# moribots/plen_ml_walk

Hardware: NVIDIA B200
Metric: PLEN env-steps/sec (higher is better)
Workload: dtype f32

## Files before the change

### plen_ml_walk_b200/csrc/plen_device.cuh

```cuda
#pragma once

#include <math.h>
#include <stdint.h>

#include "../../include/plen_b200.h"

#ifndef PLEN_HOST_EMU
#define PLEN_DEV __device__ __forceinline__
#define PLEN_DEV_NOINLINE __device__ __noinline__
namespace plen {
PLEN_DEV int lane_id() { return threadIdx.x & 31; }
PLEN_DEV float shfl(float v, int src) { return __shfl_sync(0xffffffffu, v, src); }
PLEN_DEV float shfl4(float v, int src) { return __shfl_sync(0xffffffffu, v, src, 4); }
PLEN_DEV float shfl_up(float v, int d) { return __shfl_up_sync(0xffffffffu, v, d); }
PLEN_DEV float shfl_down(float v, int d) { return __shfl_down_sync(0xffffffffu, v, d); }
PLEN_DEV float shfl_xor(float v, int m) { return __shfl_xor_sync(0xffffffffu, v, m); }
PLEN_DEV unsigned ballot(bool p) { return __ballot_sync(0xffffffffu, p); }
PLEN_DEV unsigned redux_max(unsigned v) { return __reduce_max_sync(0xffffffffu, v); }
PLEN_DEV unsigned redux_or(unsigned v) { return __reduce_or_sync(0xffffffffu, v); }
PLEN_DEV void warp_sync() { __syncwarp(); }
PLEN_DEV float f_as_u_max(float v) { return __uint_as_float(redux_max(__float_as_uint(v))); }
PLEN_DEV void sincos_(float x, float *s, float *c) { sincosf(x, s, c); }
#ifndef PLEN_FAST_RCP
#define PLEN_FAST_RCP 1
#endif
PLEN_DEV float rcp_(float x) {
#if PLEN_FAST_RCP
    float r;
    asm("rcp.approx.ftz.f32 %0, %1;" : "=f"(r) : "f"(x));
    return r;
#else
    return 1.0f / x;
#endif
}
PLEN_DEV unsigned f_bits(float v) { return __float_as_uint(v); }
PLEN_DEV int lowest_bit(unsigned m) { return __ffs((int)m) - 1; }
PLEN_DEV int highest_bit(unsigned m) { return 31 - __clz((int)m); }
PLEN_DEV int popc_(unsigned m) { return __popc(m); }
}
#endif

namespace plen {

enum {
    T_RPJ = 0, T_PPJ = 9, T_AXIS = 12, T_COM = 15, T_MASS = 18, T_INERTIA = 19, T_LOWER = 25, T_UPPER = 26,
    T_CS = 27, T_CE = 28, T_ENVLO = 29, T_ENVHI = 30,
    T_BOX_LANE = 31, T_BOX_C = 32, T_BOX_R = 35, T_BOX_H = 44, T_BOX_REST = 47, T_ROWS = 48
};

enum {
    W_U = 0,
    W_Q = 32,
    W_POS = 32,
    W_MAN = 35,
    W_EPRET = 36,
    W_QUAT = 56,
    W_CNT = 60, W_DS = 61, W_HIST = 62, W_EPT = 63,
    W_LAST = 64,
    W_SUMS = 70,
    W_ITERS = 79,
    W_SPARE = 80
};

struct DevConfig {
    float dt, inv_dt, gravity_z, motor_imp, kp_over_dt, one_minus_kd, linear_damping;
    float mu_lateral, mu_spinning, mu_rolling, restitution, rest_thresh, erp_contact_over_dt, erp_joint_over_dt;
    float linear_slop, warm, hull_margin, vmax, residual_threshold, mu_link;
    float foot_break[2];
    float foot_pts[2][4][3];
    float start_pos[3];
    int foot_lane[2];
    int substeps, reset_ticks, iterations, joint_act, max_episode_steps, auto_reset, link_contacts, n_boxes;
    int sole_manifold, n_hull[2];
    const float *hull;
    float support_tie;
};

enum {
    SR_G = 0,
    SR_B = 960,
    SR_MRHS = 1152, SR_MD = 1184, SR_LDIR = 1216, SR_LRHS = 1248, SR_VSTAR = 1280, SR_Q = 1312,
    SR_CRHS = 1344, SR_CDINV = 1408, SR_CD = 1472,
    SR_PT = 1536,
    SR_LAMC = 1568,
    SR_BASE = 1576,
    SR_WORDS = 1600
};

enum {
    XR_NX = 0,
    XR_ROWS = 16,
    XR_J = 0, XR_B = 32, XR_BB = 64, XR_RHS = 70, XR_DINV = 71, XR_D = 72, XR_ROW_WORDS = 80,
    XR_WORDS = XR_ROWS + 3 * PLEN_MAX_BOX_POINTS * XR_ROW_WORDS
};
#define PLEN_KEY_EXT 125

PLEN_DEV int nth_bit4(unsigned m, int k) {
    int r = -1, c = 0;
#pragma unroll
    for (int b = 0; b < 4; b++) {
        const bool on = (m >> b) & 1u;
        r = (on && c == k) ? b : r;
        c += on ? 1 : 0;
    }
    return r;
}

#ifndef PLEN_HOST_EMU
struct __align__(16) vec4 { float x, y, z, w; };
struct __align__(8) vec2 { float x, y; };
#define PLEN_ALIGN16 __align__(16)
#else
struct vec4 { float x, y, z, w; };
struct vec2 { float x, y; };
#define PLEN_ALIGN16
#endif

#ifndef PLEN_HOST_EMU
PLEN_DEV float gld(const float *p) {
    float v;
    asm("ld.global.f32 %0, [%1];" : "=f"(v) : "l"(p));
    return v;
}
PLEN_DEV vec4 gld4(const float *p) {
    vec4 r;
    asm("ld.global.v4.f32 {%0, %1, %2, %3}, [%4];" : "=f"(r.x), "=f"(r.y), "=f"(r.z), "=f"(r.w) : "l"(p));
    return r;
}
PLEN_DEV int gld_i(const int *p) {
    int v;
    asm("ld.global.s32 %0, [%1];" : "=r"(v) : "l"(p));
    return v;
}
PLEN_DEV int gld_u8(const uint8_t *p) {
    unsigned v;
    asm("ld.global.u8 %0, [%1];" : "=r"(v) : "l"(p));
    return (int)v;
}
#else
PLEN_DEV float gld(const float *p) { return *p; }
PLEN_DEV vec4 gld4(const float *p) { return *reinterpret_cast<const vec4 *>(p); }
PLEN_DEV int gld_i(const int *p) { return *p; }
PLEN_DEV int gld_u8(const uint8_t *p) { return *p; }
#endif

PLEN_DEV void load6(const float *row, float (&o)[6]) {
    const vec4 a = *reinterpret_cast<const vec4 *>(row);
    const vec2 b = *reinterpret_cast<const vec2 *>(row + 4);
    o[0] = a.x; o[1] = a.y; o[2] = a.z; o[3] = a.w; o[4] = b.x; o[5] = b.y;
}

struct PLEN_ALIGN16 WarpScratch {
    float st[96];
    float tw[24][8];
    float kk[24][8];
    float gg[24][8];
    float cb[32];
    float minv[24][32];
    float cp[8][4];
    union {
        float lin[12][12];
        float red[32 * 21];
    };
    float obs[32];
    float xp[PLEN_MAX_BOX_POINTS][8];
    float mn[2][28];
    float mlam[8];
};

struct LaneState {
    float u;
    float q;
    float tgt;
    float lam;
    float pos[3];
    float quat[4];
    unsigned man;
    int iters;
    float fric_s, motor_s, kp_s;
};

PLEN_DEV void mat3_mul(const float *A, const float *B, float *C) {
#pragma unroll
    for (int i = 0; i < 3; i++)
#pragma unroll
        for (int j = 0; j < 3; j++) C[3 * i + j] = A[3 * i] * B[j] + A[3 * i + 1] * B[3 + j] + A[3 * i + 2] * B[6 + j];
}
PLEN_DEV void mat3_vec(const float *A, const float *v, float *o) {
    o[0] = A[0] * v[0] + A[1] * v[1] + A[2] * v[2];
    o[1] = A[3] * v[0] + A[4] * v[1] + A[5] * v[2];
    o[2] = A[6] * v[0] + A[7] * v[1] + A[8] * v[2];
}
PLEN_DEV void cross(const float *a, const float *b, float *o) {
    o[0] = a[1] * b[2] - a[2] * b[1];
    o[1] = a[2] * b[0] - a[0] * b[2];
    o[2] = a[0] * b[1] - a[1] * b[0];
}
PLEN_DEV void quat_to_mat(const float *q, float *R) {
    const float x = q[0], y = q[1], z = q[2], w = q[3];
    R[0] = 1 - 2 * (y * y + z * z); R[1] = 2 * (x * y - w * z); R[2] = 2 * (x * z + w * y);
    R[3] = 2 * (x * y + w * z); R[4] = 1 - 2 * (x * x + z * z); R[5] = 2 * (y * z - w * x);
    R[6] = 2 * (x * z - w * y); R[7] = 2 * (y * z + w * x); R[8] = 1 - 2 * (x * x + y * y);
}
PLEN_DEV float warp_sum(float v) {
#pragma unroll
    for (int m = 16; m > 0; m >>= 1) v += shfl_xor(v, m);
    return v;
}
PLEN_DEV void warp_sum2(float &a, float &b) {
#pragma unroll
    for (int m = 16; m > 0; m >>= 1) { a += shfl_xor(a, m); b += shfl_xor(b, m); }
}

PLEN_DEV void forward_kinematics(const float *tab, int lane, float q, const float *quat, float *Rw, float *pw) {
    float R[9], p[3];
    {
        float s, c;
        sincos_(q, &s, &c);
        const float ax = tab[(T_AXIS + 0) * 32 + lane], ay = tab[(T_AXIS + 1) * 32 + lane], az = tab[(T_AXIS + 2) * 32 + lane];
        const float t = 1.0f - c;
        float Rq[9] = {t * ax * ax + c, t * ax * ay - s * az, t * ax * az + s * ay,
                       t * ax * ay + s * az, t * ay * ay + c, t * ay * az - s * ax,
                       t * ax * az - s * ay, t * ay * az + s * ax, t * az * az + c};
        float Rpj[9];
#pragma unroll
        for (int k = 0; k < 9; k++) Rpj[k] = tab[(T_RPJ + k) * 32 + lane];
        mat3_mul(Rpj, Rq, R);
#pragma unroll
        for (int k = 0; k < 3; k++) p[k] = tab[(T_PPJ + k) * 32 + lane];
    }
    const int cs = (int)tab[T_CS * 32 + lane];
#pragma unroll
    for (int d = 1; d < 8; d <<= 1) {
        float Rp[9], pp[3];
#pragma unroll
        for (int k = 0; k < 9; k++) Rp[k] = shfl_up(R[k], d);
#pragma unroll
        for (int k = 0; k < 3; k++) pp[k] = shfl_up(p[k], d);
        if (lane - d >= cs) {
            float t[3], Rn[9];
            mat3_vec(Rp, p, t);
            p[0] = pp[0] + t[0]; p[1] = pp[1] + t[1]; p[2] = pp[2] + t[2];
            mat3_mul(Rp, R, Rn);
#pragma unroll
            for (int k = 0; k < 9; k++) R[k] = Rn[k];
        }
    }
    float R0[9];
    quat_to_mat(quat, R0);
    mat3_mul(R0, R, Rw);
    mat3_vec(R0, p, pw);
}

PLEN_DEV float clampf(float x, float lo, float hi) { return fminf(fmaxf(x, lo), hi); }

PLEN_DEV void row_entries(int type, const float *a, const float *m, const float *Y, float px, float py, float pz,
                          float &J, float &B) {
    switch (type) {
        case 0: J = a[0] * py - a[1] * px + m[2]; B = Y[0] * py - Y[1] * px + Y[5]; break;
        case 1: J = a[2]; B = Y[2]; break;
        case 2: J = -a[1]; B = -Y[1]; break;
        case 3: J = a[0]; B = Y[0]; break;
        case 4: J = a[0] * pz - a[2] * px - m[1]; B = Y[0] * pz - Y[2] * px - Y[4]; break;
        default: J = a[1] * pz - a[2] * py + m[0]; B = Y[1] * pz - Y[2] * py + Y[3]; break;
    }
}

struct DebugOut { float *minv, *pos, *rot; };

PLEN_DEV_NOINLINE void box_rows(const DevConfig &cfg, const float *tab, WarpScratch &ws, int lane, float vstar, int nx, float *srx);
PLEN_DEV_NOINLINE int box_points(const DevConfig &cfg, const float *tab, WarpScratch &ws, int lane, bool touch, float cz, float rz0,
                                 float rz1, float rz2, int bl, float R0, float R1, float R2, float R3, float R4, float R5, float R6,
                                 float R7, float R8, float p0, float p1, float p2);

PLEN_DEV_NOINLINE void manifold_merge(const DevConfig &cfg, float *mn, float *lam, const float *Rf, const float *pf, const float *pos,
                                      int f, int idx);

PLEN_DEV_NOINLINE unsigned sole_manifold_contacts(const DevConfig &cfg, WarpScratch &ws, int lane, float *man, float pos0, float pos1,
                                                  float pos2, float lam_in, float R0, float R1, float R2, float R3, float R4, float R5,
                                                  float R6, float R7, float R8, float p0, float p1, float p2);

PLEN_DEV void tick_dynamics(const DevConfig &cfg, const float *tab, WarpScratch &ws, LaneState &L, int lane,
                            float *srec, uint8_t *sort_key, const DebugOut *dbg = nullptr, float *srx = nullptr,
                            float *man = nullptr) {
    const bool is_joint = lane >= 6 && lane < 24;
    const int cs = (int)tab[T_CS * 32 + lane], ce = (int)tab[T_CE * 32 + lane];
    float Rw[9], pw[3];
    forward_kinematics(tab, lane, L.q, L.quat, Rw, pw);

    float a[3] = {0, 0, 0}, m[3] = {0, 0, 0};
    if (is_joint) {
        float ax[3] = {tab[(T_AXIS + 0) * 32 + lane], tab[(T_AXIS + 1) * 32 + lane], tab[(T_AXIS + 2) * 32 + lane]};
        mat3_vec(Rw, ax, a);
        cross(pw, a, m);
    } else if (lane < 3) {
        a[lane] = 1.0f;
    } else if (lane < 6) {
        m[lane - 3] = 1.0f;
    }
    if (lane < 24) {
#pragma unroll
        for (int k = 0; k < 3; k++) { ws.tw[lane][k] = a[k]; ws.tw[lane][3 + k] = m[k]; }
    }

    const float mass = tab[T_MASS * 32 + lane];
    float h[3], Ib[6];
    {
        float com[3] = {tab[(T_COM + 0) * 32 + lane], tab[(T_COM + 1) * 32 + lane], tab[(T_COM + 2) * 32 + lane]};
        float c[3];
        mat3_vec(Rw, com, c);
        c[0] += pw[0]; c[1] += pw[1]; c[2] += pw[2];
        const float ixx = tab[(T_INERTIA + 0) * 32 + lane], iyy = tab[(T_INERTIA + 1) * 32 + lane],
                    izz = tab[(T_INERTIA + 2) * 32 + lane], ixy = tab[(T_INERTIA + 3) * 32 + lane],
                    ixz = tab[(T_INERTIA + 4) * 32 + lane], iyz = tab[(T_INERTIA + 5) * 32 + lane];
        float T[9] = {Rw[0] * ixx + Rw[1] * ixy + Rw[2] * ixz, Rw[0] * ixy + Rw[1] * iyy + Rw[2] * iyz, Rw[0] * ixz + Rw[1] * iyz + Rw[2] * izz,
                      Rw[3] * ixx + Rw[4] * ixy + Rw[5] * ixz, Rw[3] * ixy + Rw[4] * iyy + Rw[5] * iyz, Rw[3] * ixz + Rw[4] * iyz + Rw[5] * izz,
                      Rw[6] * ixx + Rw[7] * ixy + Rw[8] * ixz, Rw[6] * ixy + Rw[7] * iyy + Rw[8] * iyz, Rw[6] * ixz + Rw[7] * iyz + Rw[8] * izz};
        const float cc = c[0] * c[0] + c[1] * c[1] + c[2] * c[2];
        Ib[0] = T[0] * Rw[0] + T[1] * Rw[1] + T[2] * Rw[2] + mass * (cc - c[0] * c[0]);
        Ib[1] = T[3] * Rw[3] + T[4] * Rw[4] + T[5] * Rw[5] + mass * (cc - c[1] * c[1]);
        Ib[2] = T[6] * Rw[6] + T[7] * Rw[7] + T[8] * Rw[8] + mass * (cc - c[2] * c[2]);
        Ib[3] = T[0] * Rw[3] + T[1] * Rw[4] + T[2] * Rw[5] - mass * c[0] * c[1];
        Ib[4] = T[0] * Rw[6] + T[1] * Rw[7] + T[2] * Rw[8] - mass * c[0] * c[2];
        Ib[5] = T[3] * Rw[6] + T[4] * Rw[7] + T[5] * Rw[8] - mass * c[1] * c[2];
        h[0] = mass * c[0]; h[1] = mass * c[1]; h[2] = mass * c[2];
    }

    float V0[6];
#pragma unroll
    for (int k = 0; k < 6; k++) V0[k] = shfl(L.u, k);
    float tv[6];
#pragma unroll
    for (int k = 0; k < 3; k++) { tv[k] = is_joint ? a[k] * L.u : 0.0f; tv[3 + k] = is_joint ? m[k] * L.u : 0.0f; }
    float V[6];
#pragma unroll
    for (int k = 0; k < 6; k++) V[k] = tv[k];
#pragma unroll
    for (int d = 1; d < 8; d <<= 1) {
#pragma unroll
        for (int k = 0; k < 6; k++) {
            const float t = shfl_up(V[k], d);
            if (lane - d >= cs) V[k] += t;
        }
    }
#pragma unroll
    for (int k = 0; k < 6; k++) V[k] += V0[k];

    float ab[6];
    {
        float t1[3], t2[3], t3[3];
        cross(V, tv, t1);
        cross(V, tv + 3, t2);
        cross(V + 3, tv, t3);
#pragma unroll
        for (int k = 0; k < 3; k++) { ab[k] = t1[k]; ab[3 + k] = t2[k] + t3[k]; }
#pragma unroll
        for (int d = 1; d < 8; d <<= 1) {
#pragma unroll
            for (int k = 0; k < 6; k++) {
                const float t = shfl_up(ab[k], d);
                if (lane - d >= cs) ab[k] += t;
            }
        }
        float wv[3];
        cross(V0, V0 + 3, wv);
        ab[3] -= wv[0]; ab[4] -= wv[1]; ab[5] -= wv[2] + cfg.gravity_z;
    }

    float F[6];
    {
        float IV[6], Ia[6], t[3], t2[3];
        cross(h, V + 3, t);
        IV[0] = Ib[0] * V[0] + Ib[3] * V[1] + Ib[4] * V[2] + t[0];
        IV[1] = Ib[3] * V[0] + Ib[1] * V[1] + Ib[5] * V[2] + t[1];
        IV[2] = Ib[4] * V[0] + Ib[5] * V[1] + Ib[2] * V[2] + t[2];
        cross(h, V, t);
        IV[3] = mass * V[3] - t[0]; IV[4] = mass * V[4] - t[1]; IV[5] = mass * V[5] - t[2];
        cross(h, ab + 3, t);
        Ia[0] = Ib[0] * ab[0] + Ib[3] * ab[1] + Ib[4] * ab[2] + t[0];
        Ia[1] = Ib[3] * ab[0] + Ib[1] * ab[1] + Ib[5] * ab[2] + t[1];
        Ia[2] = Ib[4] * ab[0] + Ib[5] * ab[1] + Ib[2] * ab[2] + t[2];
        cross(h, ab, t);
        Ia[3] = mass * ab[3] - t[0]; Ia[4] = mass * ab[4] - t[1]; Ia[5] = mass * ab[5] - t[2];
        cross(V, IV, t);
        cross(V + 3, IV + 3, t2);
        F[0] = Ia[0] + t[0] + t2[0]; F[1] = Ia[1] + t[1] + t2[1]; F[2] = Ia[2] + t[2] + t2[2];
        cross(V, IV + 3, t);
        F[3] = Ia[3] + t[0]; F[4] = Ia[4] + t[1]; F[5] = Ia[5] + t[2];
        if (cfg.linear_damping != 0.0f && mass > 0.0f) {
            float c[3] = {h[0] / mass, h[1] / mass, h[2] / mass}, vc[3], fd[3], nd[3];
            cross(V, c, t);
            vc[0] = V[3] + t[0]; vc[1] = V[4] + t[1]; vc[2] = V[5] + t[2];
            const float nv = sqrtf(vc[0] * vc[0] + vc[1] * vc[1] + vc[2] * vc[2]);
            const float k = cfg.linear_damping * mass * (1.0f + nv);
            fd[0] = -k * vc[0]; fd[1] = -k * vc[1]; fd[2] = -k * vc[2];
            cross(c, fd, nd);
            F[0] -= nd[0]; F[1] -= nd[1]; F[2] -= nd[2];
            F[3] -= fd[0]; F[4] -= fd[1]; F[5] -= fd[2];
        }
    }

    float mc = mass, hc[3] = {h[0], h[1], h[2]}, Ic[6] = {Ib[0], Ib[1], Ib[2], Ib[3], Ib[4], Ib[5]};
    float Fc[6] = {F[0], F[1], F[2], F[3], F[4], F[5]};
#pragma unroll
    for (int d = 1; d < 8; d <<= 1) {
        const bool take = is_joint && (lane + d <= ce);
        float t;
        t = shfl_down(mc, d); if (take) mc += t;
#pragma unroll
        for (int k = 0; k < 3; k++) { t = shfl_down(hc[k], d); if (take) hc[k] += t; }
#pragma unroll
        for (int k = 0; k < 6; k++) { t = shfl_down(Ic[k], d); if (take) Ic[k] += t; }
#pragma unroll
        for (int k = 0; k < 6; k++) { t = shfl_down(Fc[k], d); if (take) Fc[k] += t; }
    }
    float mt, ht[3], It[6], Ft[6];
    {
        const bool root = (lane == 0) || (is_joint && lane == cs);
        const unsigned roots = ballot(root);
        const int ord = popc_(roots & ((1u << lane) - 1u)), n_roots = popc_(roots);
        if (root) {
            float *dst = ws.red + 16 * ord;
            dst[0] = mc; dst[1] = hc[0]; dst[2] = hc[1]; dst[3] = hc[2];
#pragma unroll
            for (int k = 0; k < 6; k++) { dst[4 + k] = Ic[k]; dst[10 + k] = Fc[k]; }
        }
        warp_sync();
        float acc[16];
#pragma unroll
        for (int v = 0; v < 16; v++) acc[v] = 0.0f;
        for (int r = 0; r < n_roots; r++) {
#pragma unroll
            for (int q = 0; q < 4; q++) {
                const vec4 x = *reinterpret_cast<const vec4 *>(ws.red + 16 * r + 4 * q);
                acc[4 * q] += x.x; acc[4 * q + 1] += x.y; acc[4 * q + 2] += x.z; acc[4 * q + 3] += x.w;
            }
        }
        mt = acc[0]; ht[0] = acc[1]; ht[1] = acc[2]; ht[2] = acc[3];
#pragma unroll
        for (int k = 0; k < 6; k++) { It[k] = acc[4 + k]; Ft[k] = acc[10 + k]; }
        warp_sync();
    }

    float Cl = 0.0f, fM[6] = {0, 0, 0, 0, 0, 0};
    if (is_joint) {
        Cl = a[0] * Fc[0] + a[1] * Fc[1] + a[2] * Fc[2] + m[0] * Fc[3] + m[1] * Fc[4] + m[2] * Fc[5];
        float t[3];
        cross(hc, m, t);
        fM[0] = Ic[0] * a[0] + Ic[3] * a[1] + Ic[4] * a[2] + t[0];
        fM[1] = Ic[3] * a[0] + Ic[1] * a[1] + Ic[5] * a[2] + t[1];
        fM[2] = Ic[4] * a[0] + Ic[5] * a[1] + Ic[2] * a[2] + t[2];
        cross(hc, a, t);
        fM[3] = mc * m[0] - t[0]; fM[4] = mc * m[1] - t[1]; fM[5] = mc * m[2] - t[2];
    } else if (lane < 6) {
        Cl = Ft[lane];
    }
    ws.cb[lane] = Cl;

    float Mrow[6], Krow[6];
    const int off = lane - cs;
    {
        if (lane < 24) {
#pragma unroll
            for (int k = 0; k < 6; k++) ws.kk[lane][k] = fM[k];
        }
        warp_sync();
#pragma unroll
        for (int d = 0; d < 6; d++) {
            const int j = cs + d;
            float v = (d == off) ? 1.0f : 0.0f;
            if (is_joint && j <= ce) {
                float r6[6];
                if (d <= off) {
                    load6(ws.tw[j], r6);
                    v = r6[0] * fM[0] + r6[1] * fM[1] + r6[2] * fM[2] + r6[3] * fM[3] + r6[4] * fM[4] + r6[5] * fM[5];
                } else {
                    load6(ws.kk[j], r6);
                    v = a[0] * r6[0] + a[1] * r6[1] + a[2] * r6[2] + m[0] * r6[3] + m[1] * r6[4] + m[2] * r6[5];
                }
            }
            Mrow[d] = v;
        }
#pragma unroll
        for (int k = 0; k < 6; k++) Krow[k] = fM[k];
        warp_sync();
    }
#pragma unroll
    for (int k = 0; k < 6; k++) {
        const bool act = is_joint && (cs + k <= ce);
        const int src = act ? cs + k : lane;
        float pr[6], pk[6];
#pragma unroll
        for (int d = 0; d < 6; d++) pr[d] = shfl(Mrow[d], src);
#pragma unroll
        for (int d = 0; d < 6; d++) pk[d] = shfl(Krow[d], src);
        if (act) {
            const float inv = rcp_(pr[k]);
            if (off == k) {
#pragma unroll
                for (int d = 0; d < 6; d++) Mrow[d] = (d == k) ? inv : pr[d] * inv;
#pragma unroll
                for (int d = 0; d < 6; d++) Krow[d] = pk[d] * inv;
            } else {
                const float f = Mrow[k] * inv;
#pragma unroll
                for (int d = 0; d < 6; d++) Mrow[d] = (d == k) ? -f : Mrow[d] - f * pr[d];
#pragma unroll
                for (int d = 0; d < 6; d++) Krow[d] -= f * pk[d];
            }
        }
    }

    {
        int idx = 0;
#pragma unroll
        for (int r = 0; r < 6; r++)
#pragma unroll
            for (int c = r; c < 6; c++) { ws.red[lane * 21 + idx] = is_joint ? fM[r] * Krow[c] : 0.0f; idx++; }
        warp_sync();
        if (lane < 21) {
            float s = 0.0f;
            for (int j = 6; j < 24; j++) s += ws.red[j * 21 + lane];
            ws.red[lane] = s;
        }
    }
    warp_sync();
    float R[6];
    {
        float M00[6][6] = {{It[0], It[3], It[4], 0.0f, -ht[2], ht[1]},
                           {It[3], It[1], It[5], ht[2], 0.0f, -ht[0]},
                           {It[4], It[5], It[2], -ht[1], ht[0], 0.0f},
                           {0.0f, ht[2], -ht[1], mt, 0.0f, 0.0f},
                           {-ht[2], 0.0f, ht[0], 0.0f, mt, 0.0f},
                           {ht[1], -ht[0], 0.0f, 0.0f, 0.0f, mt}};
        float S[6][6];
        int idx = 0;
#pragma unroll
        for (int r = 0; r < 6; r++)
#pragma unroll
            for (int c = r; c < 6; c++) {
                const float v = M00[r][c] - ws.red[idx];
                S[r][c] = v; S[c][r] = v; idx++;
            }
#pragma unroll
        for (int c = 0; c < 6; c++) {
            float v = S[0][c];
#pragma unroll
            for (int r = 1; r < 6; r++) v = (lane == r) ? S[r][c] : v;
            R[c] = v;
        }
#pragma unroll
        for (int k = 0; k < 6; k++) {
            const float inv = rcp_(R[k]);
            float P[6];
#pragma unroll
            for (int j = 0; j < 6; j++) P[j] = shfl((j == k) ? inv : R[j] * inv, k);
            const float f = R[k];
            const bool piv = lane == k;
#pragma unroll
            for (int j = 0; j < 6; j++) {
                const float elim = (j == k) ? -(f * P[k]) : R[j] - f * P[j];
                R[j] = piv ? P[j] : elim;
            }
        }
    }
    warp_sync();
    if (lane < 6) {
#pragma unroll
        for (int k = 0; k < 6; k++) ws.gg[lane][k] = R[k];
    }
    warp_sync();
    float G[6];
    {
        float Si[6][6];
#pragma unroll
        for (int b = 0; b < 6; b++)
#pragma unroll
            for (int c = 0; c < 6; c++) Si[b][c] = ws.gg[b][c];
#pragma unroll
        for (int c = 0; c < 6; c++) {
            float s = 0.0f;
#pragma unroll
            for (int b = 0; b < 6; b++) s += Krow[b] * Si[b][c];
            G[c] = is_joint ? s : 0.0f;
        }
    }
    warp_sync();
    if (lane < 24) {
#pragma unroll
        for (int k = 0; k < 6; k++) { ws.kk[lane][k] = is_joint ? Krow[k] : 0.0f; ws.gg[lane][k] = G[k]; }
    }
    warp_sync();
    if (lane < 24) {
#pragma unroll
        for (int k = 0; k < 6; k++) ws.minv[k][lane] = is_joint ? -G[k] : R[k];
        const float *ggl = &ws.gg[0][is_joint ? 0 : lane];
#pragma unroll 6
        for (int j = 6; j < 24; j++) {
            float r6[6];
            load6(ws.kk[j], r6);
            const float s = G[0] * r6[0] + G[1] * r6[1] + G[2] * r6[2] + G[3] * r6[3] + G[4] * r6[4] + G[5] * r6[5];
            ws.minv[j][lane] = is_joint ? s : -ggl[j * 8];
        }
        if (is_joint) {
#pragma unroll
            for (int d = 0; d < 6; d++)
                if (cs + d <= ce) ws.minv[cs + d][lane] += Mrow[d];
        }
    }
    warp_sync();

    if (dbg != nullptr && lane < 24) {
        if (dbg->minv) for (int j = 0; j < 24; j++) dbg->minv[lane * 24 + j] = ws.minv[j][lane];
        if (dbg->pos) for (int k = 0; k < 3; k++) dbg->pos[lane * 3 + k] = pw[k] + L.pos[k];
        if (dbg->rot) for (int k = 0; k < 9; k++) dbg->rot[lane * 9 + k] = Rw[k];
    }

    float vstar = 0.0f;
    if (lane < 24) {
        float acc = 0.0f;
        for (int j = 0; j < 24; j++) acc += ws.minv[j][lane] * ws.cb[j];
        vstar = clampf(L.u - cfg.dt * acc, -cfg.vmax, cfg.vmax);
    }

    unsigned man_new;
    if (cfg.sole_manifold && man != nullptr) {
        man_new = sole_manifold_contacts(cfg, ws, lane, man, L.pos[0], L.pos[1], L.pos[2], L.lam, Rw[0], Rw[1], Rw[2], Rw[3], Rw[4],
                                         Rw[5], Rw[6], Rw[7], Rw[8], pw[0], pw[1], pw[2]);
        L.man = man_new;
        L.lam = (lane >= 24) ? ws.mlam[lane - 24] : L.lam;
    } else {
        const int i = lane - 24, f = (lane >= 28) ? 1 : 0;
        const int src = cfg.foot_lane[f];
        float Rf[9], pf[3];
#pragma unroll
        for (int k = 0; k < 9; k++) Rf[k] = shfl(Rw[k], src);
#pragma unroll
        for (int k = 0; k < 3; k++) pf[k] = shfl(pw[k], src);
        bool in = false;
        if (lane >= 24) {
            const float *pt = cfg.foot_pts[f][i & 3];
            float w[3];
            mat3_vec(Rf, pt, w);
            w[0] += pf[0]; w[1] += pf[1]; w[2] += pf[2];
            const float dist = (L.pos[2] + w[2]) - cfg.hull_margin;
            in = dist <= cfg.foot_break[f];
            ws.cp[i][0] = w[0]; ws.cp[i][1] = w[1]; ws.cp[i][2] = w[2] - cfg.hull_margin; ws.cp[i][3] = dist;
            const bool was = (L.man >> i) & 1u;
            if (!in || !was) L.lam = 0.0f;
        }
        man_new = ballot(in) >> 24;
        L.man = man_new;
    }
    warp_sync();

    int nx = 0;
    if (cfg.link_contacts && srx != nullptr) {
        const int bl = (int)tab[T_BOX_LANE * 32 + lane];
        const float r20 = shfl(Rw[6], bl), r21 = shfl(Rw[7], bl), r22 = shfl(Rw[8], bl), pz = shfl(pw[2], bl);
        float rz[3], az[3];
#pragma unroll
        for (int k = 0; k < 3; k++) {
            rz[k] = r20 * tab[(T_BOX_R + k) * 32 + lane] + r21 * tab[(T_BOX_R + 3 + k) * 32 + lane] + r22 * tab[(T_BOX_R + 6 + k) * 32 + lane];
            az[k] = rz[k] * tab[(T_BOX_H + k) * 32 + lane];
        }
        const float cz = L.pos[2] + pz + r20 * tab[(T_BOX_C + 0) * 32 + lane] + r21 * tab[(T_BOX_C + 1) * 32 + lane] +
                         r22 * tab[(T_BOX_C + 2) * 32 + lane];
        const bool touch = lane < cfg.n_boxes && cz - (fabsf(az[0]) + fabsf(az[1]) + fabsf(az[2])) <= 0.0f;
        if (ballot(touch))
            nx = box_points(cfg, tab, ws, lane, touch, cz, rz[0], rz[1], rz[2], bl, Rw[0], Rw[1], Rw[2], Rw[3], Rw[4], Rw[5], Rw[6],
                            Rw[7], Rw[8], pw[0], pw[1], pw[2]);
    }
    const bool ext = nx > 0;

    float Y[2][6];
#pragma unroll
    for (int f = 0; f < 2; f++) {
        const int fl = cfg.foot_lane[f], fcs = fl - 5;
#pragma unroll
        for (int k = 0; k < 6; k++) Y[f][k] = 0.0f;
        if ((((man_new >> (4 * f)) & 0xFu) || (f == 0 && ext)) && lane < 24) {
#pragma unroll
            for (int k = 0; k < 6; k++) Y[f][k] = ws.minv[k][lane];
            for (int j = fcs; j <= fl; j++) {
                const float w = ws.minv[j][lane];
                float r6[6];
                load6(ws.tw[j], r6);
#pragma unroll
                for (int k = 0; k < 6; k++) Y[f][k] += w * r6[k];
            }
        }
    }

    float m_dinv = 0.0f, m_rhs = 0.0f, l_rhs = 0.0f, l_dir = 0.0f;
    if (is_joint) {
        const float m_d = ws.minv[lane][lane];
        m_dinv = (m_d > 1.1920929e-7f) ? rcp_(m_d) : 0.0f;
        const float desired = cfg.kp_over_dt * L.kp_s * (L.tgt - L.q) + cfg.one_minus_kd * vstar;
        m_rhs = (m_dinv > 0.0f) ? (desired - vstar) : 0.0f;
        const float lo = tab[T_LOWER * 32 + lane], hi = tab[T_UPPER * 32 + lane];
        const float pen_lo = L.q - lo, pen_hi = hi - L.q;
        if (m_dinv > 0.0f) {
            if (pen_lo <= 0.0f) { l_dir = 1.0f; l_rhs = -pen_lo * cfg.erp_joint_over_dt - vstar; }
            else if (pen_hi <= 0.0f) { l_dir = -1.0f; l_rhs = -pen_hi * cfg.erp_joint_over_dt + vstar; }
        }
    }
    ws.obs[lane] = vstar;
    if (lane < 24) {
#pragma unroll
        for (int k = 0; k < 6; k++) { ws.kk[lane][k] = Y[0][k]; ws.gg[lane][k] = Y[1][k]; }
    }
    warp_sync();
    if (man_new || ext) {
        if (lane < 12) {
            const int f = (lane >= 6) ? 1 : 0, k = lane - 6 * f, fl = cfg.foot_lane[f];
            float acc = 0.0f;
#pragma unroll
            for (int l = 0; l < 6; l++) acc += ws.tw[l][k] * ws.obs[l];
#pragma unroll
            for (int l = 0; l < 6; l++) acc += ws.tw[fl - 5 + l][k] * ws.obs[fl - 5 + l];
            ws.st[W_SPARE + lane] = acc;
        }
        for (int e = lane; e < 144; e += 32) {
            const int row = e / 12, col = e - 12 * row;
            const int fa = row / 6, a6 = row - 6 * fa, fb = col / 6, b6 = col - 6 * fb;
            const float(*Yb)[8] = fb ? ws.gg : ws.kk;
            float acc = Yb[a6][b6];
            const int fl = cfg.foot_lane[fa];
            for (int j = fl - 5; j <= fl; j++) acc += ws.tw[j][a6] * Yb[j][b6];
            ws.lin[row][col] = acc;
        }
        warp_sync();
    }

    {
        const int i = lane;
        const bool ij = i < 18, ic = (i >= 18 && i < 24) || i >= 26;
        const int fa = (i >= 26) ? 1 : 0, a6 = fa ? i - 26 : i - 18;
        const float(*Ya)[8] = fa ? ws.gg : ws.kk;
        float *G = srec + SR_G;
        ws.obs[lane] = m_dinv;
        warp_sync();
        {
            const float *b1 = ij ? &ws.minv[6][6 + i] : (ic ? &Ya[6][a6] : &ws.cb[0]);
            const int st1 = ij ? 32 : (ic ? 8 : 0);
            const bool on1 = ij || ic;
#pragma unroll
            for (int c = 0; c < 18; c++) {
                const float v = b1[c * st1];
                G[c * 32 + lane] = on1 ? v * ws.obs[6 + c] : 0.0f;
            }
        }
        {
            const bool on2 = ij || (ic && (man_new || ext));
            const float *b2 = ij ? &ws.kk[6 + i][0] : (on2 ? &ws.lin[fa * 6 + a6][0] : &ws.cb[0]);
            const int jump = ij ? (int)(&ws.gg[0][0] - &ws.kk[0][0]) - 6 : 0, st2 = on2 ? 1 : 0;
#pragma unroll
            for (int c = 18; c < 30; c++) {
                const int fb = (c >= 24) ? 1 : 0;
                const float v = b2[(c - 18) * st2 + (fb ? jump : 0)];
                G[c * 32 + lane] = on2 ? v : 0.0f;
            }
        }
        const int src = ij ? 6 + i : 0;
        const float s_rhs = shfl(m_rhs, src), s_dinv = shfl(m_dinv, src), s_ldir = shfl(l_dir, src),
                    s_lrhs = shfl(l_rhs, src), s_vs = shfl(vstar, src), s_q = shfl(L.q, src),
                    s_d = shfl(is_joint ? ws.minv[lane][lane] : 0.0f, src);
        float *Bm = srec + SR_B;
        {
            const float *b3 = ij ? &ws.minv[6 + i][0] : (ic ? &Ya[0][a6] : &ws.cb[0]);
            const int st3 = ij ? 1 : (ic ? 8 : 0);
            const float sc3 = ij ? s_dinv : (ic ? 1.0f : 0.0f);
#pragma unroll
            for (int k = 0; k < 6; k++) Bm[k * 32 + lane] = (ij || ic) ? b3[k * st3] * sc3 : 0.0f;
        }
        srec[SR_MRHS + lane] = ij ? s_rhs : 0.0f;
        srec[SR_MD + lane] = (ij && s_dinv > 0.0f) ? s_d : 0.0f;
        srec[SR_LDIR + lane] = ij ? s_ldir : 0.0f;
        srec[SR_LRHS + lane] = ij ? s_lrhs : 0.0f;
        srec[SR_VSTAR + lane] = ij ? s_vs : 0.0f;
        srec[SR_Q + lane] = ij ? s_q : 0.0f;
    }

#pragma unroll
    for (int half = 0; half < 2; half++) {
        const int f = half, g = lane & 7, comp = g - 2;
        const int pb = nth_bit4((man_new >> (4 * f)) & 15u, lane >> 3);
        const int p = 4 * f + (pb < 0 ? 0 : pb);
        const bool valid = comp >= 0 && pb >= 0;
        float rhs = 0.0f, dinv = 0.0f, d = 0.0f;
        if (valid) {
            const float px = ws.cp[p][0], py = ws.cp[p][1], pz = ws.cp[p][2];
            int i0 = comp, i1 = comp, i2 = comp;
            float c0 = 1.0f, c1 = 0.0f, c2 = 0.0f;
            if (comp == 3) { i0 = 1; i1 = 2; i2 = 3; c0 = pz; c1 = -py; c2 = 1.0f; }
            else if (comp == 4) { i0 = 0; i1 = 2; i2 = 4; c0 = -pz; c1 = px; c2 = 1.0f; }
            else if (comp == 5) { i0 = 0; i1 = 1; i2 = 5; c0 = py; c1 = -px; c2 = 1.0f; }
            const int o = 6 * f;
            d = c0 * (c0 * ws.lin[o + i0][o + i0] + c1 * ws.lin[o + i0][o + i1] + c2 * ws.lin[o + i0][o + i2]) +
                c1 * (c0 * ws.lin[o + i1][o + i0] + c1 * ws.lin[o + i1][o + i1] + c2 * ws.lin[o + i1][o + i2]) +
                c2 * (c0 * ws.lin[o + i2][o + i0] + c1 * ws.lin[o + i2][o + i1] + c2 * ws.lin[o + i2][o + i2]);
            dinv = (d > 1.1920929e-7f) ? rcp_(d) : 0.0f;
            const float *vsf = &ws.st[W_SPARE + 6 * f];
            const float v0 = vsf[i0], v1 = vsf[i1], v2 = vsf[i2];
            const float rel = c0 * v0 + c1 * v1 + c2 * v2;
            if (comp == 5) {
                const float pdist = ws.cp[p][3] + cfg.linear_slop;
                float rest = (fabsf(rel) < cfg.rest_thresh) ? 0.0f : cfg.restitution * -rel;
                rest = fmaxf(rest, 0.0f);
                float velerr = rest - rel, poserr = 0.0f;
                if (pdist > 0.0f) velerr -= pdist * cfg.inv_dt; else poserr = -pdist * cfg.erp_contact_over_dt;
                rhs = (poserr + velerr) * dinv;
            } else {
                rhs = -rel * dinv;
                if (comp < 3) {
                    const float mu = (comp == 2) ? cfg.mu_spinning : cfg.mu_rolling;
                    if (!(mu > 0.0f)) { dinv = 0.0f; rhs = 0.0f; d = 0.0f; }
                }
            }
        }
        srec[SR_CRHS + 32 * half + lane] = rhs;
        srec[SR_CDINV + 32 * half + lane] = dinv;
        srec[SR_CD + 32 * half + lane] = d;
    }
    {
        const int q = lane >> 2, pb = nth_bit4((man_new >> (4 * (q >> 2))) & 15u, q & 3);
        srec[SR_PT + lane] = (pb >= 0) ? ws.cp[4 * (q >> 2) + pb][lane & 3] : 0.0f;
        const int q2 = lane & 7, pb2 = nth_bit4((man_new >> (4 * (q2 >> 2))) & 15u, q2 & 3);
        const float lc = shfl(L.lam, 24 + 4 * (q2 >> 2) + (pb2 < 0 ? 0 : pb2));
        if (lane >= 24) srec[SR_LAMC + q2] = (pb2 >= 0) ? lc : 0.0f;
    }
    if (lane < 6) srec[SR_BASE + lane] = vstar;
    if (lane < 3) srec[SR_BASE + 6 + lane] = L.pos[lane];
    if (lane < 4) srec[SR_BASE + 9 + lane] = L.quat[lane];
    if (lane == 0) {
        srec[SR_BASE + 13] = (float)man_new;
        srec[SR_BASE + 14] = L.fric_s;
        srec[SR_BASE + 15] = L.motor_s;
        const int n0 = popc_(man_new & 15u), n1 = popc_((man_new >> 4) & 15u);
        if (sort_key) *sort_key = ext ? (uint8_t)(PLEN_KEY_EXT + nx - 1) : (uint8_t)((n0 > n1 ? n0 : n1) * 25 + n0 * 5 + n1);
    }
    warp_sync();
    if (ext) box_rows(cfg, tab, ws, lane, vstar, nx, srx);
}

PLEN_DEV_NOINLINE unsigned sole_manifold_contacts(const DevConfig &cfg, WarpScratch &ws, int lane, float *man, float pos0, float pos1,
                                                  float pos2, float lam_in, float R0, float R1, float R2, float R3, float R4, float R5,
                                                  float R6, float R7, float R8, float p0, float p1, float p2) {
    const float Rw[9] = {R0, R1, R2, R3, R4, R5, R6, R7, R8}, pw[3] = {p0, p1, p2}, pos[3] = {pos0, pos1, pos2};
    unsigned man_new = 0;
    float lam_out = 0.0f;
    if (lane < 24) { ws.mn[0][lane] = man[lane]; ws.mn[1][lane] = man[24 + lane]; }
    if (lane < 2) ws.mn[lane][24] = man[48 + lane];
    if (lane >= 24) ws.mlam[lane - 24] = lam_in;
    warp_sync();
    int idx2[2];
#pragma unroll
    for (int f = 0; f < 2; f++) {
        const int src = cfg.foot_lane[f];
        const float r6 = shfl(Rw[6], src), r7 = shfl(Rw[7], src), r8 = shfl(Rw[8], src);
        const float *hv = cfg.hull + (size_t)f * PLEN_MAX_HULL * 3;
        const int nh = cfg.n_hull[f];
        float z[PLEN_MAX_HULL / 32];
        float zmin = 3.0e38f;
#pragma unroll
        for (int j = 0; j < PLEN_MAX_HULL / 32; j++) {
            const int i = lane + 32 * j;
            z[j] = 3.0e38f;
            if (i < nh) z[j] = r6 * hv[3 * i] + r7 * hv[3 * i + 1] + r8 * hv[3 * i + 2];
            zmin = fminf(zmin, z[j]);
        }
#pragma unroll
        for (int d = 16; d > 0; d >>= 1) zmin = fminf(zmin, shfl_xor(zmin, d));
        const float zlim = zmin + cfg.support_tie;
        int idx = 0x7fffffff;
#pragma unroll
        for (int j = PLEN_MAX_HULL / 32 - 1; j >= 0; j--)
            if (z[j] <= zlim && lane + 32 * j < nh) idx = lane + 32 * j;
        idx2[f] = 0x7fffffff - (int)redux_max((unsigned)(0x7fffffff - idx));
    }
    {
        const int f = lane & 1, src = cfg.foot_lane[f];
        float Rf[9], pf[3];
#pragma unroll
        for (int k = 0; k < 9; k++) Rf[k] = shfl(Rw[k], src);
#pragma unroll
        for (int k = 0; k < 3; k++) pf[k] = shfl(pw[k], src);
        if (lane < 2) manifold_merge(cfg, ws.mn[f], ws.mlam + 4 * f, Rf, pf, pos, f, f ? idx2[1] : idx2[0]);
        warp_sync();
    }
    {
        const int i = lane - 24, f = (lane >= 28) ? 1 : 0, k = i & 3;
        const int src = cfg.foot_lane[f];
        float Rf[9], pf[3];
#pragma unroll
        for (int q = 0; q < 9; q++) Rf[q] = shfl(Rw[q], src);
#pragma unroll
        for (int q = 0; q < 3; q++) pf[q] = shfl(pw[q], src);
        bool in = false;
        if (lane >= 24) {
            in = k < (int)ws.mn[f][24];
            float w[3] = {0.0f, 0.0f, 0.0f};
            if (in) { mat3_vec(Rf, &ws.mn[f][3 * k], w); w[0] += pf[0]; w[1] += pf[1]; w[2] += pf[2]; }
            ws.cp[i][0] = w[0]; ws.cp[i][1] = w[1]; ws.cp[i][2] = w[2];
            ws.cp[i][3] = in ? (pos[2] + w[2]) - ws.mn[f][12 + 3 * k + 2] : 0.0f;
            lam_out = in ? ws.mlam[i] : 0.0f;
        }
        man_new = ballot(in) >> 24;
    }
    warp_sync();
    if (lane < 24) { man[lane] = ws.mn[0][lane]; man[24 + lane] = ws.mn[1][lane]; }
    if (lane < 2) man[48 + lane] = ws.mn[lane][24];
    warp_sync();
    if (lane >= 24) ws.mlam[lane - 24] = lam_out;
    warp_sync();
    return man_new;
}

PLEN_DEV_NOINLINE void manifold_merge(const DevConfig &cfg, float *mn, float *lam, const float *Rf, const float *pf, const float *pos,
                                      int f, int idx) {
    float *loc = mn, *pln = mn + 12;
    int n = (int)mn[24];
    const float thr = cfg.foot_break[f];
    const float fx = pos[0] + pf[0], fy = pos[1] + pf[1], fz = pos[2] + pf[2];
    if (idx >= 0 && idx < cfg.n_hull[f]) {
        const float *v = cfg.hull + ((size_t)f * PLEN_MAX_HULL + idx) * 3;
        const float la[3] = {v[0] - cfg.hull_margin * Rf[6], v[1] - cfg.hull_margin * Rf[7], v[2] - cfg.hull_margin * Rf[8]};
        float t[3];
        mat3_vec(Rf, la, t);
        const float pa[3] = {fx + t[0], fy + t[1], fz + t[2]};
        const float dist = pa[2];
        if (dist < thr) {
            int slot = -1;
            float nearest = thr * thr;
            for (int k = 0; k < n; k++) {
                const float e0 = loc[3 * k] - la[0], e1 = loc[3 * k + 1] - la[1], e2 = loc[3 * k + 2] - la[2];
                const float dd = e0 * e0 + e1 * e1 + e2 * e2;
                if (dd < nearest) { nearest = dd; slot = k; }
            }
            if (slot < 0) {
                if (n < 4) { slot = n; n = n + 1; lam[slot] = 0.0f; }
                else {
                    int deepest = -1;
                    float maxpen = dist;
                    for (int k = 0; k < 4; k++) {
                        const float zk = fz + Rf[6] * loc[3 * k] + Rf[7] * loc[3 * k + 1] + Rf[8] * loc[3 * k + 2];
                        if (zk < maxpen) { deepest = k; maxpen = zk; }
                    }
                    float best = -1.0f;
                    slot = 0;
                    for (int k = 0; k < 4; k++) {
                        float res = 0.0f;
                        if (k != deepest) {
                            const int o0 = (k == 0) ? 1 : 0, o1 = (k <= 1) ? 2 : 1, o2 = (k <= 2) ? 3 : 2;
                            const float a[3] = {la[0] - loc[3 * o0], la[1] - loc[3 * o0 + 1], la[2] - loc[3 * o0 + 2]};
                            const float b[3] = {loc[3 * o2] - loc[3 * o1], loc[3 * o2 + 1] - loc[3 * o1 + 1], loc[3 * o2 + 2] - loc[3 * o1 + 2]};
                            float c[3];
                            cross(a, b, c);
                            res = c[0] * c[0] + c[1] * c[1] + c[2] * c[2];
                        }
                        if (res > best) { best = res; slot = k; }
                    }
                    lam[slot] = 0.0f;
                }
            }
            loc[3 * slot] = la[0]; loc[3 * slot + 1] = la[1]; loc[3 * slot + 2] = la[2];
            pln[3 * slot] = pa[0]; pln[3 * slot + 1] = pa[1]; pln[3 * slot + 2] = 0.0f;
        }
    }
    for (int k = n - 1; k >= 0; k--) {
        float t[3];
        mat3_vec(Rf, loc + 3 * k, t);
        const float dist = (fz + t[2]) - pln[3 * k + 2];
        const float dx = pln[3 * k] - (fx + t[0]), dy = pln[3 * k + 1] - (fy + t[1]);
        if (dist > thr || dx * dx + dy * dy > thr * thr) {
            const int last = n - 1;
            if (k != last) {
                for (int c = 0; c < 3; c++) { loc[3 * k + c] = loc[3 * last + c]; pln[3 * k + c] = pln[3 * last + c]; }
                lam[k] = lam[last];
            }
            lam[last] = 0.0f;
            n = last;
        }
    }
    mn[24] = (float)n;
}

PLEN_DEV_NOINLINE int box_points(const DevConfig &cfg, const float *tab, WarpScratch &ws, int lane, bool touch, float cz, float rz0,
                                 float rz1, float rz2, int bl, float R0, float R1, float R2, float R3, float R4, float R5, float R6,
                                 float R7, float R8, float p0, float p1, float p2) {
    const float Rw[9] = {R0, R1, R2, R3, R4, R5, R6, R7, R8}, pw[3] = {p0, p1, p2};
    const float rz[3] = {rz0, rz1, rz2};
    float az[3];
#pragma unroll
    for (int k = 0; k < 3; k++) az[k] = rz[k] * tab[(T_BOX_H + k) * 32 + lane];
    int nx = 0;
    const int ks = (fabsf(rz[1]) > fabsf(rz[0])) ? ((fabsf(rz[2]) > fabsf(rz[1])) ? 2 : 1) : ((fabsf(rz[2]) > fabsf(rz[0])) ? 2 : 0);
    const float zs = (ks == 0) ? az[0] : ((ks == 1) ? az[1] : az[2]);
    const float zi = (ks == 0) ? az[1] : ((ks == 1) ? az[2] : az[0]);
    const float zj = (ks == 0) ? az[2] : ((ks == 1) ? az[0] : az[1]);
    float depth[4];
    unsigned cand = 0;
#pragma unroll
    for (int v = 0; v < 4; v++) {
        const float vz = cz - fabsf(zs) + ((v & 1) ? zi : -zi) + ((v & 2) ? zj : -zj);
        depth[v] = -vz;
        if (touch && depth[v] >= 0.0f) cand |= 1u << v;
    }
    unsigned mine = 0;
    for (int q = 0; q < PLEN_MAX_BOX_POINTS; q++) {
        float bd = -1.0f;
        int bv = 0;
#pragma unroll
        for (int v = 0; v < 4; v++)
            if (((cand & ~mine) >> v) & 1u) { if (depth[v] > bd) { bd = depth[v]; bv = v; } }
        const unsigned key = (bd >= 0.0f) ? f_bits(bd) + 1u : 0u;
        const unsigned best = redux_max(key);
        if (best == 0u) break;
        if (lane == lowest_bit(ballot(key == best))) mine |= 1u << bv;
        nx++;
    }
    if (nx) {
        int below = 0;
#pragma unroll
        for (int b = 0; b < 4; b++) below += popc_(ballot((mine >> b) & 1u) & ((1u << lane) - 1u));
        float Rb[9], pb[3];
#pragma unroll
        for (int k = 0; k < 9; k++) Rb[k] = shfl(Rw[k], bl);
#pragma unroll
        for (int k = 0; k < 3; k++) pb[k] = shfl(pw[k], bl);
        if (mine) {
            float ax[3][3], c[3];
#pragma unroll
            for (int k = 0; k < 3; k++) {
                const float h = tab[(T_BOX_H + k) * 32 + lane];
#pragma unroll
                for (int r = 0; r < 3; r++)
                    ax[k][r] = (Rb[3 * r] * tab[(T_BOX_R + k) * 32 + lane] + Rb[3 * r + 1] * tab[(T_BOX_R + 3 + k) * 32 + lane] +
                                Rb[3 * r + 2] * tab[(T_BOX_R + 6 + k) * 32 + lane]) * h;
            }
#pragma unroll
            for (int r = 0; r < 3; r++)
                c[r] = pb[r] + Rb[3 * r] * tab[(T_BOX_C + 0) * 32 + lane] + Rb[3 * r + 1] * tab[(T_BOX_C + 1) * 32 + lane] +
                       Rb[3 * r + 2] * tab[(T_BOX_C + 2) * 32 + lane];
            const float sg = (zs > 0.0f) ? -1.0f : 1.0f;
            int slot = below;
#pragma unroll
            for (int v = 0; v < 4; v++) {
                if (!((mine >> v) & 1u)) continue;
                const float si = (v & 1) ? 1.0f : -1.0f, sj = (v & 2) ? 1.0f : -1.0f;
#pragma unroll
                for (int r = 0; r < 3; r++) {
                    const float as_ = (ks == 0) ? ax[0][r] : ((ks == 1) ? ax[1][r] : ax[2][r]);
                    const float ai_ = (ks == 0) ? ax[1][r] : ((ks == 1) ? ax[2][r] : ax[0][r]);
                    const float aj_ = (ks == 0) ? ax[2][r] : ((ks == 1) ? ax[0][r] : ax[1][r]);
                    ws.xp[slot][r] = c[r] + sg * as_ + si * ai_ + sj * aj_;
                }
                ws.xp[slot][3] = depth[v];
                ws.xp[slot][4] = (float)bl;
                ws.xp[slot][5] = tab[T_BOX_REST * 32 + lane];
                slot++;
            }
        }
        warp_sync();
    }
    return nx;
}

PLEN_DEV_NOINLINE void box_rows(const DevConfig &cfg, const float *tab, WarpScratch &ws, int lane, float vstar, int nx, float *srx) {
    float *Jg = ws.red, *Bg = ws.red + 96;
    const int flR = cfg.foot_lane[0], flL = cfg.foot_lane[1];
    if (lane == 0) srx[XR_NX] = (float)nx;
    for (int q = 0; q < nx; q++) {
        const float px = ws.xp[q][0], py = ws.xp[q][1], pz = ws.xp[q][2], depth = ws.xp[q][3];
        const int bl = (int)ws.xp[q][4];
        const float restf = ws.xp[q][5];
        const int bcs = (int)tab[T_CS * 32 + bl];
        const bool sup = lane < 6 || (bl >= 6 && lane >= bcs && lane <= bl);
        float a[3] = {0, 0, 0}, m[3] = {0, 0, 0};
        if (lane < 24) {
#pragma unroll
            for (int k = 0; k < 3; k++) { a[k] = ws.tw[lane][k]; m[k] = ws.tw[lane][3 + k]; }
        }
        float jg[3];
        jg[0] = a[0] * py - a[1] * px + m[2];
        jg[1] = a[0] * pz - a[2] * px - m[1];
        jg[2] = a[1] * pz - a[2] * py + m[0];
        warp_sync();
#pragma unroll
        for (int r = 0; r < 3; r++) { jg[r] = (sup && lane < 24) ? jg[r] : 0.0f; Jg[32 * r + lane] = jg[r]; }
        warp_sync();
        float bg[3] = {0, 0, 0};
        if (lane < 24) {
            for (int j = 0; j < 6; j++) {
                const float w = ws.minv[j][lane];
#pragma unroll
                for (int r = 0; r < 3; r++) bg[r] += w * Jg[32 * r + j];
            }
            if (bl >= 6)
                for (int j = bcs; j <= bl; j++) {
                    const float w = ws.minv[j][lane];
#pragma unroll
                    for (int r = 0; r < 3; r++) bg[r] += w * Jg[32 * r + j];
                }
        }
#pragma unroll
        for (int r = 0; r < 3; r++) Bg[32 * r + lane] = bg[r];
        warp_sync();
#pragma unroll
        for (int r = 0; r < 3; r++) {
            float d = jg[r] * bg[r], rel = jg[r] * vstar;
            warp_sum2(d, rel);
            const float dinv = (d > 1.1920929e-7f) ? rcp_(d) : 0.0f;
            float rhs;
            if (r == 0) {
                const float pdist = -depth + cfg.linear_slop;
                float rest = (fabsf(rel) < cfg.rest_thresh) ? 0.0f : cfg.restitution * restf * -rel;
                rest = fmaxf(rest, 0.0f);
                float velerr = rest - rel, poserr = 0.0f;
                if (pdist > 0.0f) velerr -= pdist * cfg.inv_dt; else poserr = -pdist * cfg.erp_contact_over_dt;
                rhs = (poserr + velerr) * dinv;
            } else {
                rhs = -rel * dinv;
            }
            const int i = lane;
            float jx = 0.0f, bx = 0.0f;
            const float *jr = Jg + 32 * r, *br = Bg + 32 * r;
            if (i < 18) {
                const int j = 6 + i;
                jx = jr[j];
                if (j >= flR - 5 && j <= flR) {
#pragma unroll
                    for (int k = 0; k < 6; k++) jx -= jr[k] * ws.tw[j][k];
                }
                bx = br[j];
            } else if (i < 24 || i >= 26) {
                const int c = (i < 24) ? i - 18 : i - 26, fl = (i < 24) ? flR : flL;
                jx = (i < 24) ? jr[c] : 0.0f;
                bx = br[c];
                for (int j = fl - 5; j <= fl; j++) bx += ws.tw[j][c] * br[j];
            }
            float *row = srx + XR_ROWS + (3 * q + r) * XR_ROW_WORDS;
            row[XR_J + lane] = jx;
            row[XR_B + lane] = bx;
            if (lane < 6) row[XR_BB + lane] = br[lane];
            if (lane == 0) { row[XR_RHS] = rhs; row[XR_DINV] = dinv; row[XR_D] = d; }
        }
    }
    warp_sync();
}

}
```

Baseline: 17.75 million.

## Use packed f32x2 FMA/mul and shared-memory reads for per-lane dynamics math

Replaces scalar multiply and FMA loops in the inertia elimination, Gaussian elimination, G product and Y accumulation with the packed fma.rn.f32x2 and mul.rn.f32x2 instructions, so each instruction handles two lanes of data. Replaces shuffles of base velocity with shared-memory loads from the warp scratch state. Turns lane-dependent branches into predicated selects to cut divergence, and reads position and quaternion from scratch instead of per-lane registers. The scratch reads assume ws.st already holds up-to-date state. The mov.b64 packing may add register moves that cancel the savings.

```diff
diff --git a/plen_ml_walk_b200/csrc/plen_device.cuh b/plen_ml_walk_b200/csrc/plen_device.cuh
--- a/plen_ml_walk_b200/csrc/plen_device.cuh
+++ b/plen_ml_walk_b200/csrc/plen_device.cuh
@@ -144,6 +144,25 @@
 PLEN_DEV int gld_u8(const uint8_t *p) { return *p; }
 #endif
 
+PLEN_DEV void fma_x2(float &o0, float &o1, float a0, float a1, float b0, float b1, float c0, float c1) {
+#ifndef PLEN_HOST_EMU
+    asm("{ .reg .b64 ra, rb, rc; mov.b64 ra, {%2, %3}; mov.b64 rb, {%4, %5}; mov.b64 rc, {%6, %7};\n\t"
+        "fma.rn.f32x2 ra, ra, rb, rc; mov.b64 {%0, %1}, ra; }"
+        : "=f"(o0), "=f"(o1) : "f"(a0), "f"(a1), "f"(b0), "f"(b1), "f"(c0), "f"(c1));
+#else
+    o0 = fmaf(a0, b0, c0); o1 = fmaf(a1, b1, c1);
+#endif
+}
+PLEN_DEV void mul_x2(float &o0, float &o1, float a0, float a1, float b0, float b1) {
+#ifndef PLEN_HOST_EMU
+    asm("{ .reg .b64 ra, rb; mov.b64 ra, {%2, %3}; mov.b64 rb, {%4, %5};\n\t"
+        "mul.rn.f32x2 ra, ra, rb; mov.b64 {%0, %1}, ra; }"
+        : "=f"(o0), "=f"(o1) : "f"(a0), "f"(a1), "f"(b0), "f"(b1));
+#else
+    o0 = a0 * b0; o1 = a1 * b1;
+#endif
+}
+
 PLEN_DEV void load6(const float *row, float (&o)[6]) {
     const vec4 a = *reinterpret_cast<const vec4 *>(row);
     const vec2 b = *reinterpret_cast<const vec2 *>(row + 4);
@@ -293,10 +312,9 @@
         float ax[3] = {tab[(T_AXIS + 0) * 32 + lane], tab[(T_AXIS + 1) * 32 + lane], tab[(T_AXIS + 2) * 32 + lane]};
         mat3_vec(Rw, ax, a);
         cross(pw, a, m);
-    } else if (lane < 3) {
-        a[lane] = 1.0f;
-    } else if (lane < 6) {
-        m[lane - 3] = 1.0f;
+    } else {
+#pragma unroll
+        for (int k = 0; k < 3; k++) { a[k] = (lane == k) ? 1.0f : 0.0f; m[k] = (lane == 3 + k) ? 1.0f : 0.0f; }
     }
     if (lane < 24) {
 #pragma unroll
@@ -327,8 +345,7 @@
     }
 
     float V0[6];
-#pragma unroll
-    for (int k = 0; k < 6; k++) V0[k] = shfl(L.u, k);
+    load6(ws.st + W_U, V0);
     float tv[6];
 #pragma unroll
     for (int k = 0; k < 3; k++) { tv[k] = is_joint ? a[k] * L.u : 0.0f; tv[3 + k] = is_joint ? m[k] * L.u : 0.0f; }
@@ -452,8 +469,9 @@
         fM[2] = Ic[4] * a[0] + Ic[5] * a[1] + Ic[2] * a[2] + t[2];
         cross(hc, a, t);
         fM[3] = mc * m[0] - t[0]; fM[4] = mc * m[1] - t[1]; fM[5] = mc * m[2] - t[2];
-    } else if (lane < 6) {
-        Cl = Ft[lane];
+    } else {
+#pragma unroll
+        for (int k = 0; k < 6; k++) Cl = (lane == k) ? Ft[k] : Cl;
     }
     ws.cb[lane] = Cl;
 
@@ -498,15 +516,19 @@
             const float inv = rcp_(pr[k]);
             if (off == k) {
 #pragma unroll
-                for (int d = 0; d < 6; d++) Mrow[d] = (d == k) ? inv : pr[d] * inv;
-#pragma unroll
-                for (int d = 0; d < 6; d++) Krow[d] = pk[d] * inv;
+                for (int d = 0; d < 6; d += 2) {
+                    mul_x2(Mrow[d], Mrow[d + 1], pr[d], pr[d + 1], inv, inv);
+                    mul_x2(Krow[d], Krow[d + 1], pk[d], pk[d + 1], inv, inv);
+                }
+                Mrow[k] = inv;
             } else {
                 const float f = Mrow[k] * inv;
 #pragma unroll
-                for (int d = 0; d < 6; d++) Mrow[d] = (d == k) ? -f : Mrow[d] - f * pr[d];
-#pragma unroll
-                for (int d = 0; d < 6; d++) Krow[d] -= f * pk[d];
+                for (int d = 0; d < 6; d += 2) {
+                    fma_x2(Mrow[d], Mrow[d + 1], -f, -f, pr[d], pr[d + 1], Mrow[d], Mrow[d + 1]);
+                    fma_x2(Krow[d], Krow[d + 1], -f, -f, pk[d], pk[d + 1], Krow[d], Krow[d + 1]);
+                }
+                Mrow[k] = -f;
             }
         }
     }
@@ -514,9 +536,14 @@
     {
         int idx = 0;
 #pragma unroll
-        for (int r = 0; r < 6; r++)
-#pragma unroll
-            for (int c = r; c < 6; c++) { ws.red[lane * 21 + idx] = is_joint ? fM[r] * Krow[c] : 0.0f; idx++; }
+        for (int r = 0; r < 6; r++) {
+            float p[6];
+            if (r & 1) p[r] = fM[r] * Krow[r];
+#pragma unroll
+            for (int c = (r + 1) & ~1; c < 6; c += 2) mul_x2(p[c], p[c + 1], fM[r], fM[r], Krow[c], Krow[c + 1]);
+#pragma unroll
+            for (int c = r; c < 6; c++) { ws.red[lane * 21 + idx] = is_joint ? p[c] : 0.0f; idx++; }
+        }
         warp_sync();
         if (lane < 21) {
             float s = 0.0f;
@@ -554,14 +581,18 @@
             const float inv = rcp_(R[k]);
             float P[6];
 #pragma unroll
-            for (int j = 0; j < 6; j++) P[j] = shfl((j == k) ? inv : R[j] * inv, k);
+            for (int j = 0; j < 6; j += 2) mul_x2(P[j], P[j + 1], R[j], R[j + 1], inv, inv);
+            P[k] = inv;
+#pragma unroll
+            for (int j = 0; j < 6; j++) P[j] = shfl(P[j], k);
             const float f = R[k];
             const bool piv = lane == k;
-#pragma unroll
-            for (int j = 0; j < 6; j++) {
-                const float elim = (j == k) ? -(f * P[k]) : R[j] - f * P[j];
-                R[j] = piv ? P[j] : elim;
-            }
+            float elim[6];
+#pragma unroll
+            for (int j = 0; j < 6; j += 2) fma_x2(elim[j], elim[j + 1], -f, -f, P[j], P[j + 1], R[j], R[j + 1]);
+            elim[k] = -(f * P[k]);
+#pragma unroll
+            for (int j = 0; j < 6; j++) R[j] = piv ? P[j] : elim[j];
         }
     }
     warp_sync();
@@ -578,11 +609,12 @@
 #pragma unroll
             for (int c = 0; c < 6; c++) Si[b][c] = ws.gg[b][c];
 #pragma unroll
-        for (int c = 0; c < 6; c++) {
-            float s = 0.0f;
-#pragma unroll
-            for (int b = 0; b < 6; b++) s += Krow[b] * Si[b][c];
-            G[c] = is_joint ? s : 0.0f;
+        for (int c = 0; c < 6; c += 2) {
+            float s0 = 0.0f, s1 = 0.0f;
+#pragma unroll
+            for (int b = 0; b < 6; b++) fma_x2(s0, s1, Krow[b], Krow[b], Si[b][c], Si[b][c + 1], s0, s1);
+            G[c] = is_joint ? s0 : 0.0f;
+            G[c + 1] = is_joint ? s1 : 0.0f;
         }
     }
     warp_sync();
@@ -612,7 +644,7 @@
 
     if (dbg != nullptr && lane < 24) {
         if (dbg->minv) for (int j = 0; j < 24; j++) dbg->minv[lane * 24 + j] = ws.minv[j][lane];
-        if (dbg->pos) for (int k = 0; k < 3; k++) dbg->pos[lane * 3 + k] = pw[k] + L.pos[k];
+        if (dbg->pos) for (int k = 0; k < 3; k++) dbg->pos[lane * 3 + k] = pw[k] + ws.st[W_POS + k];
         if (dbg->rot) for (int k = 0; k < 9; k++) dbg->rot[lane * 9 + k] = Rw[k];
     }
 
@@ -625,7 +657,7 @@
 
     unsigned man_new;
     if (cfg.sole_manifold && man != nullptr) {
-        man_new = sole_manifold_contacts(cfg, ws, lane, man, L.pos[0], L.pos[1], L.pos[2], L.lam, Rw[0], Rw[1], Rw[2], Rw[3], Rw[4],
+        man_new = sole_manifold_contacts(cfg, ws, lane, man, ws.st[W_POS], ws.st[W_POS + 1], ws.st[W_POS + 2], L.lam, Rw[0], Rw[1], Rw[2], Rw[3], Rw[4],
                                          Rw[5], Rw[6], Rw[7], Rw[8], pw[0], pw[1], pw[2]);
         L.man = man_new;
         L.lam = (lane >= 24) ? ws.mlam[lane - 24] : L.lam;
@@ -687,7 +719,7 @@
                 float r6[6];
                 load6(ws.tw[j], r6);
 #pragma unroll
-                for (int k = 0; k < 6; k++) Y[f][k] += w * r6[k];
+                for (int k = 0; k < 6; k += 2) fma_x2(Y[f][k], Y[f][k + 1], w, w, r6[k], r6[k + 1], Y[f][k], Y[f][k + 1]);
             }
         }
     }
@@ -830,9 +862,10 @@
         const float lc = shfl(L.lam, 24 + 4 * (q2 >> 2) + (pb2 < 0 ? 0 : pb2));
         if (lane >= 24) srec[SR_LAMC + q2] = (pb2 >= 0) ? lc : 0.0f;
     }
-    if (lane < 6) srec[SR_BASE + lane] = vstar;
-    if (lane < 3) srec[SR_BASE + 6 + lane] = L.pos[lane];
-    if (lane < 4) srec[SR_BASE + 9 + lane] = L.quat[lane];
+    {
+        const float b = (lane < 6) ? vstar : ws.st[(lane < 9) ? W_POS - 6 + lane : W_QUAT - 9 + lane];
+        if (lane < 13) srec[SR_BASE + lane] = b;
+    }
     if (lane == 0) {
         srec[SR_BASE + 13] = (float)man_new;
         srec[SR_BASE + 14] = L.fric_s;
```

Result: faster. 18.01 million, median of 6 (+1.5%).
